# makgyver/gossipy

Hardware: AMD Instinct MI355X
Metric: node-rounds/sec (gossip rounds/sec x nodes, Hegedus-2021 logreg) (higher is better)
Workload: dtype fp32; 1 GPU; model=logreg-57x2 (Hegedus-2021), nodes=1000, nodes_per_gpu=1000, delta=100, protocol=push, mode=merge_update, parallelism=node-sharded gossip over RCCL/xGMI (dp1)

## Files before the change

### gossipy_amd/csrc/scheduler.cpp

```cpp

#include <pybind11/numpy.h>
#include <pybind11/pybind11.h>
#include <pybind11/stl.h>

#include <algorithm>
#include <cmath>
#include <cstdint>
#include <map>
#include <memory>
#include <deque>
#include <functional>
#include <unordered_map>
#include <chrono>
#include <cstdio>
#include <unordered_set>
#include <vector>

#include "round_layout.h"
#include "round_prefetch.h"
#include "round_source.h"

namespace py = pybind11;


// ... 669 lines not shown
        if (ring_mask_) {
            size_t sl = (size_t)t & ring_mask_;
            if (ring_tick_[sl] == t) {
                out.swap(ring_[sl]);
                ring_tick_[sl] = INT64_MIN;
            }
        } else {
            auto it = pending_.find(t);
            if (it != pending_.end()) {
                out = std::move(it->second);
                pending_.erase(it);
            }
        }
        return out;
    }
    int64_t slot_reuse_lag_ = 32;
    std::deque<std::pair<int64_t, int32_t>> reuse_q_;
    int64_t next_slot_ = 0;
    std::vector<int32_t> slot_owner_;

    int32_t alloc_slot(int32_t owner, int64_t t)
    {
        int32_t s;
        if (!reuse_q_.empty() && reuse_q_.front().first + slot_reuse_lag_ <= t) {
            s = reuse_q_.front().second;
            reuse_q_.pop_front();
        } else {
            s = (int32_t)next_slot_++;
            if (next_slot_ > (int64_t)slot_owner_.size())
                slot_owner_.resize(slot_owner_.size() * 2);
// ... 196 lines not shown
    RoundData rd;
    int64_t &sent = rd.sent, &failed = rd.failed, &total_size = rd.total_size;
    auto &snap_nodes = rd.snap_nodes, &snap_slots = rd.snap_slots,
         &snap_tptr = rd.snap_tptr;
    auto &recv_nodes = rd.recv_nodes, &recv_tptr = rd.recv_tptr,
         &recv_nptr = rd.recv_nptr;
    auto &del_slots = rd.del_slots, &del_owners = rd.del_owners,
         &reply_slots = rd.reply_slots, &del_pids = rd.del_pids;
    auto &pull_nodes = rd.pull_nodes, &pull_slots = rd.pull_slots,
         &pull_tptr = rd.pull_tptr;
    auto &rep_nodes = rd.rep_nodes, &rep_tptr = rd.rep_tptr,
         &rep_nptr = rd.rep_nptr;
    auto &rep_slots = rd.rep_slots, &rep_owners = rd.rep_owners,
         &rep_pids = rd.rep_pids;

    std::vector<double> online(n_);
    std::vector<int32_t> firing;
    firing.reserve(64);

    for (int64_t t = t0; t < t1; ++t) {
        std::vector<int32_t> freed;

        firing.clear();
        if (sync_) {
            firing = fire_buckets_[t % delta_];
        } else {
            for (int64_t i = 0; i < n_; ++i)
                if (t % deltas_[i] == 0) firing.push_back((int32_t)i);
        }

        size_t n_f = firing.size();
        if (n_f) {
            Stream gp(stream_key(seed_, PEER, (uint64_t)t, 0));
            std::vector<int32_t> peers(n_f);
            if (indptr_.empty()) {
                for (size_t j = 0; j < n_f; ++j) {
                    int64_t draw = gp.integers(0, n_ - 1);
                    peers[j] = (int32_t)(draw + (draw >= firing[j] ? 1 : 0));
                }
            } else {
                std::vector<double> u(n_f);
                for (size_t j = 0; j < n_f; ++j) u[j] = gp.rnd();
                for (size_t j = 0; j < n_f; ++j) {
                    int64_t s = indptr_[firing[j]];
                    int64_t deg = indptr_[firing[j] + 1] - s;
                    peers[j] = (int32_t)indices_[s + (int64_t)std::floor(
                                                          u[j] * (double)deg)];
                }
            }
            std::vector<double> drop_u(n_f, 1.0);
            if (drop_ > 0.0) {
                Stream gdrop(stream_key(seed_, DROP, (uint64_t)t, 0));
                for (size_t j = 0; j < n_f; ++j) drop_u[j] = gdrop.rnd();
            }
            int64_t msize = (proto_ == PULL) ? 1 : model_size_;
            std::vector<int64_t> delays(n_f);
            {
                Stream gdl(stream_key(seed_, DELAY, (uint64_t)t, 0));
                for (size_t j = 0; j < n_f; ++j) delays[j] = delay_for(gdl, msize);
            }
            std::vector<int32_t> pids(n_f, -1);
            if (n_parts_ > 0) {
                Stream gpt(stream_key(seed_, PART, (uint64_t)t, 0));
                for (size_t j = 0; j < n_f; ++j)
                    pids[j] = (int32_t)gpt.integers(0, n_parts_);
            } else if (sampled_) {
                Stream gsm(stream_key(seed_, SAMPLE, (uint64_t)t, 0));
                for (size_t j = 0; j < n_f; ++j)
                    pids[j] = (int32_t)gsm.integers(0, (int64_t)1 << 31);
            }
            for (size_t j = 0; j < n_f; ++j) {
                int32_t sender = firing[j], receiver = peers[j];
                bool is_pull = proto_ == PULL;
                int32_t slot = -1;
                if (!is_pull) {
                    slot = alloc_slot(sender, t);
                    snap_nodes.push_back(sender);
                    snap_slots.push_back(slot);
                }
                sent += 1;
                total_size += msize;
                if (drop_u[j] >= drop_) {
                    int64_t due = t + delays[j];
                    int32_t rf = (proto_ == PUSH_PULL) ? -2 : -1;
                    pend_push(due, {receiver, slot, rf, is_pull, sender, pids[j]});
                } else {
                    failed += 1;
                    if (slot >= 0) freed.push_back(slot);
                }
            }
        }
        snap_tptr.push_back((int32_t)snap_nodes.size());

        if (online_ < 1.0) {
            Stream go(stream_key(seed_, ONLINE, (uint64_t)t, 0));
            for (int64_t i = 0; i < n_; ++i) online[i] = go.rnd();
        }
        std::vector<Msg> due = pend_take(t);
        std::vector<int32_t> order;
        ev_pool_.clear(); row_head_.clear(); row_tail_.clear();
        const int64_t st_main = 2 * t;
        auto row_append = [&](int64_t stamp, int32_t node, int32_t a,
                              int32_t b, int32_t c, int32_t d) {
            int32_t e = (int32_t)ev_pool_.size();
            ev_pool_.push_back({a, b, c, d, -1});
            if (row_stamp_[node] != stamp) {
                row_stamp_[node] = stamp;
                row_idx_[node] = (int32_t)order.size();
                order.push_back(node);
                row_head_.push_back(e);
                row_tail_.push_back(e);
            } else {
                ev_pool_[row_tail_[row_idx_[node]]].next = e;
                row_tail_[row_idx_[node]] = e;
// ... 27 lines not shown
            freed.push_back(m.slot);
        }
        for (size_t ri = 0; ri < order.size(); ++ri) {
            recv_nodes.push_back(order[ri]);
            for (int32_t e = row_head_[ri]; e >= 0; e = ev_pool_[e].next) {
                del_slots.push_back(ev_pool_[e].v0);
                reply_slots.push_back(ev_pool_[e].v1);
                del_owners.push_back(ev_pool_[e].v2);
                del_pids.push_back(ev_pool_[e].v3);
            }
            recv_nptr.push_back((int32_t)del_slots.size());
        }
        recv_tptr.push_back((int32_t)recv_nodes.size());
        pull_tptr.push_back((int32_t)pull_nodes.size());

        std::vector<Msg> rep_due = pend_take(t);
        std::vector<int32_t> rorder;
        ev_pool_.clear(); row_head_.clear(); row_tail_.clear();
        const int64_t st_rep = 2 * t + 1;
        auto rep_append = [&](int32_t node, int32_t a, int32_t b, int32_t c) {
            int32_t e = (int32_t)ev_pool_.size();
            ev_pool_.push_back({a, b, c, 0, -1});
            if (row_stamp_[node] != st_rep) {
                row_stamp_[node] = st_rep;
                row_idx_[node] = (int32_t)rorder.size();
                rorder.push_back(node);
                row_head_.push_back(e);
                row_tail_.push_back(e);
            } else {
                ev_pool_[row_tail_[row_idx_[node]]].next = e;
                row_tail_[row_idx_[node]] = e;
            }
// ... 9 lines not shown
        }
        for (size_t ri = 0; ri < rorder.size(); ++ri) {
            rep_nodes.push_back(rorder[ri]);
            for (int32_t e = row_head_[ri]; e >= 0; e = ev_pool_[e].next) {
                rep_slots.push_back(ev_pool_[e].v0);
                rep_owners.push_back(ev_pool_[e].v1);
                rep_pids.push_back(ev_pool_[e].v2);
            }
            rep_nptr.push_back((int32_t)rep_slots.size());
        }
        rep_tptr.push_back((int32_t)rep_nodes.size());

        for (int32_t s : freed) reuse_q_.emplace_back(t, s);
    }

    rd.n_slots = next_slot_;
    if (sampling_eval_ > 0) {
        Stream g(stream_key(seed_, EVAL, (uint64_t)(t1 - 1), 0));
        int64_t k = std::max<int64_t>((int64_t)(n_ * sampling_eval_), 1);
        rd.eval_nodes.resize(k);
        for (int64_t i = 0; i < k; ++i) rd.eval_nodes[i] = g.integers(0, n_);
    }
    return rd;
}

void NativeScheduler::pack_generated(RoundData& rd, int64_t n_nodes)
{
    rd.packed = pack_round_compute(
        rd.snap_nodes, rd.snap_slots, rd.snap_tptr, rd.recv_nodes,
        rd.recv_nptr, rd.recv_tptr, rd.del_slots, rd.reply_slots,
// ... 543 lines not shown
```

### gossipy_amd/engine/runner.py

```python

from __future__ import annotations

import os
from typing import List, Optional, Tuple

import numpy as np
import torch
import torch.distributed as dist

from .. import LOG
from ..core import CreateModelMode
from ..simul import SimulationEventSender
from .arena import DataArena, NodeStateArena, SlotPool
from .backend import make_backend
from .metrics import binary_margin_metrics, classification_metrics_shared
from .rng import RandomTape
from .schedule import (
    EngineConfig,
    RoundSchedule,
    Scheduler,
    TickPhase,
    TokenizedScheduler,
    make_scheduler,
)
# ... 1149 lines not shown
            return None
        st, d = self.state, self.data
        key = (
            name, tuple(plan), id(self.scheduler),
            *(t.data_ptr() for t in (st.params, st.ages, d.x, d.y, d.counts,
                                     d.gx, d.gy)),
        )
        if getattr(self, "_rd_key", None) != key:
            self._rd = self.backend.ext.RoundDriver(
                st.params, st.ages, self.pool.slots, self.pool.slot_ages,
                d.x, d.y, d.counts, d.gx, d.gy, name, tuple(plan),
                self.scheduler.round_source(),
                eval_all=not self.cfg.sampling_eval > 0,
                mapped_metrics=env.get("GOSSIPY_RD_NO_MAPPED_EVAL") != "1",
                side_upload=env.get("GOSSIPY_RD_NO_SIDE_UPLOAD") != "1",
            )
            self._rd_key = key
            self._rd_pool = self.pool.slots
        elif self._rd_pool is not self.pool.slots:
            self._rd.set_pool(self.pool.slots, self.pool.slot_ages)
            self._rd_pool = self.pool.slots
        return self._rd

    def _driver_round(self, drv, r: int) -> None:
        res = drv.step(r)
        if res[4] < 0:
            self.pool.ensure(res[3])
            drv.set_pool(self.pool.slots, self.pool.slot_ages)
            self._rd_pool = self.pool.slots
            res = drv.step(r)
# ... 446 lines not shown
```

### gossipy_amd/ops/hip/gossip_kernels.hip

```cpp

#include <torch/extension.h>
#include <pybind11/numpy.h>
#include <ATen/hip/HIPContext.h>
#include <hip/hip_runtime.h>
#include <hip/hip_cooperative_groups.h>

#include <array>
#include <atomic>
#include <chrono>
#include <deque>
#include <stdexcept>
#include <string>
#include <vector>

#include "round_check.h"
#include "round_layout.h"
#include "round_ring.h"
#include "round_source.h"

#define DEV_INLINE __device__ __forceinline__

constexpr int KMAX = 16;
constexpr int WAVE = 64;

// ... 189 lines not shown
            qv[u] = q ? q[s * qs] : 0.f;
        }
        if (q) {
#pragma unroll
            for (int u = 0; u < CH; ++u)
                if (s0 + u < m) g = fmaf(pv[u], qv[u], g);
        } else {
#pragma unroll
            for (int u = 0; u < CH; ++u)
                if (s0 + u < m) g += pv[u];
        }
    }
    return g;
}

template <bool BIG = false>
DEV_INLINE void logreg_update(const LogregArgs& a, int node, int c, float* W,
                              float* xb, float* dz, int& age,
                              int prestaged = 0)
{
    int tid = threadIdx.x;
    if (c == 0) return;
    int bsz = (a.bs == 0) ? c : min(a.bs, c);
    const float* Xn = a.X + (long)node * a.Smax * a.d;
    const float* Yn = a.Y + (long)node * a.Smax;
    int xb_valid = prestaged;
    for (int ep = 0; ep < a.epochs; ++ep) {
        for (int s0 = 0; s0 < c; s0 += bsz) {
            int m = min(bsz, c - s0);
            float yv = (tid < m) ? Yn[s0 + tid] : 0.f;
            if (!xb_valid) copy_row(xb, Xn + (long)s0 * a.d, m * a.d);
            xb_valid = (c <= bsz);
            __syncthreads();
            for (int pr = tid; pr < m * a.k; pr += blockDim.x) {
                int s = pr / a.k, kk = pr - s * a.k;
                dz[pr] = dot_chain(W[a.k * a.d + kk],
                                   W + kk * a.d, xb + s * a.d, a.d);
            }
            __syncthreads();
            auto dz_row = [&](int s, float y) __attribute__((always_inline)) {
                float* zs = dz + s * a.k;
                float amax = -1e30f;
                for (int kk = 0; kk < a.k; ++kk) {
                    float sg = 1.0f / (1.0f + __expf(-zs[kk]));
                    zs[kk] = sg;
                    amax = fmaxf(amax, sg);
                }
                float sum = 0.f;
                for (int kk = 0; kk < a.k; ++kk) sum += __expf(zs[kk] - amax);
                int yi = (int)y;
                float inv = 1.0f / sum;
                for (int kk = 0; kk < a.k; ++kk) {
                    float sg = zs[kk];
                    float pk = __expf(sg - amax);
                    float g = pk * inv - (kk == yi ? 1.0f : 0.0f);
                    zs[kk] = (g / m) * sg * (1.0f - sg);
                }
            };
            if (tid < m) dz_row(tid, yv);
            if constexpr (BIG) {
                for (int s = tid + blockDim.x; s < m; s += blockDim.x)
                    dz_row(s, Yn[s0 + s]);
            }
            __syncthreads();
            for (int e = tid; e < a.k * a.d; e += blockDim.x) {
                int kk = e / a.d, dd = e - kk * a.d;
                float g = col_chain(dz + kk, a.k, xb + dd, a.d, m);
                if (a.wd != 0.f) g += a.wd * W[e];
                W[e] -= a.lr * g;
            }
            for (int e = tid; e < a.k; e += blockDim.x) {
                float g = col_chain(dz + e, a.k, nullptr, 0, m);
                W[a.k * a.d + e] -= a.lr * g;
            }
            __syncthreads();
            age += 1;
        }
    }
}

template <bool LIM, bool BIG = false>
DEV_INLINE void logreg_process_node(const LogregArgs& a, int i)
{
    int node = a.nodes[i];
    int tid = threadIdx.x;
    int c = a.counts[node];
    extern __shared__ float sm[];
    float* W = sm;
    float* W2 = W + a.D;
    float* xb = W2 + a.D;
    int bsmax = (a.bs == 0) ? a.Smax : min(a.bs, a.Smax);
    float* dz = xb + bsmax * a.d;

    int j0 = a.update_only ? 0 : a.ptr[i];
    int j1 = a.update_only ? 0 : a.ptr[i + 1];
    if (!a.update_only && j1 > j0 && a.mode == MODE_MERGE_UPDATE &&
// ... 28 lines not shown
        constexpr int PRE = 8;
        float pre[PRE];
        int pre_age = 0;
        int npre = min(a.D, PRE * (int)blockDim.x);
        auto issue_pre = [&](int j) {
            if (j < j1 && !(a.dmodes && a.dmodes[j])) {
                const float* srow2 = a.slots + (long)a.dslots[j] * a.D;
                for (int u = 0; u < PRE; ++u) {
                    int e = tid + u * (int)blockDim.x;
                    pre[u] = (e < a.D) ? srow2[e] : 0.f;
                }
                pre_age = a.slot_ages[a.dslots[j]];
            }
        };
        issue_pre(j0 + 1);
        logreg_update<BIG>(a, node, c, W, xb, dz, age, 1);
        int rs0 = a.rslots ? a.rslots[j0] : -1;
        if (rs0 >= 0) {
            copy_row(a.slots + (long)rs0 * a.D, W, a.D);
            if (tid == 0) a.slot_ages[rs0] = age;
            __syncthreads();
        }
        for (int j = j0 + 1; j < j1; ++j) {
            int slot2 = a.dslots[j];
            const float* srow2 = a.slots + (long)slot2 * a.D;
            int md = (a.dmodes && a.dmodes[j]) ? MODE_PASS : a.mode;
            if (md == MODE_MERGE_UPDATE) {
                if constexpr (LIM) {
                    LimRule r = lim_rule(age, pre_age, a.lim);
                    if (r.br == LIM_ADOPT) {
                        for (int u = 0; u < PRE; ++u) {
// ... 10 lines not shown
                                   [&](float w, float s) {
                                       return r.m1 * w + r.m2 * s;
                                   });
                    }
                } else {
                    for (int u = 0; u < PRE; ++u) {
                        int e = tid + u * (int)blockDim.x;
                        if (e < a.D) W[e] = 0.5f * (W[e] + pre[u]);
                    }
                    merge_rows(W + npre, srow2 + npre, a.D - npre,
                               [](float w, float s) { return 0.5f * (w + s); });
                }
                age = max(age, pre_age);
                __syncthreads();
                issue_pre(j + 1);
                logreg_update<BIG>(a, node, c, W, xb, dz, age, xb_keep);
            } else {
                copy_row(W, srow2, a.D);
                age = a.slot_ages[slot2];
                __syncthreads();
                issue_pre(j + 1);
            }
            int rs2 = a.rslots ? a.rslots[j] : -1;
            if (rs2 >= 0) {
                copy_row(a.slots + (long)rs2 * a.D, W, a.D);
                if (tid == 0) a.slot_ages[rs2] = age;
                __syncthreads();
            }
        }
        __syncthreads();
        copy_row(a.params + (long)node * a.D, W, a.D);
        if (tid == 0) a.ages[node] = age;
        return;
    }

    copy_row(W, a.params + (long)node * a.D, a.D);
    __syncthreads();
    int age = a.ages[node];

    if (a.update_only) {
        logreg_update<BIG>(a, node, c, W, xb, dz, age);
    } else {
        for (int j = a.ptr[i]; j < a.ptr[i + 1]; ++j) {
            int slot = a.dslots[j];
            const float* srow = a.slots + (long)slot * a.D;
            int sage = a.slot_ages[slot];
            int md = (a.dmodes && a.dmodes[j]) ? MODE_PASS : a.mode;
            if (md == MODE_MERGE_UPDATE) {
                if constexpr (LIM) {
                    lim_merge_row(lim_rule(age, sage, a.lim), W, srow, a.D);
                } else {
                    merge_rows(W, srow, a.D, [](float w, float s) {
                        return 0.5f * (w + s);
                    });
                }
                age = max(age, sage);
                __syncthreads();
                logreg_update<BIG>(a, node, c, W, xb, dz, age);
            } else if (md == MODE_UPDATE) {
                copy_row(W, srow, a.D);
                age = sage;
                __syncthreads();
                logreg_update<BIG>(a, node, c, W, xb, dz, age);
            } else if (md == MODE_UPDATE_MERGE) {
                logreg_update<BIG>(a, node, c, W, xb, dz, age);
                copy_row(W2, srow, a.D);
                __syncthreads();
                int age2 = sage;
                logreg_update<BIG>(a, node, c, W2, xb, dz, age2);
                if constexpr (LIM) {
                    lim_merge_row(lim_rule(age, age2, a.lim), W, W2, a.D);
                } else {
                    for (int e = tid; e < a.D; e += blockDim.x)
                        W[e] = 0.5f * (W[e] + W2[e]);
                }
                age = max(age, age2);
                __syncthreads();
            } else {
                copy_row(W, srow, a.D);
                age = sage;
                __syncthreads();
            }
            int rs = a.rslots ? a.rslots[j] : -1;
            if (rs >= 0) {
// ... 18 lines not shown
tick_logreg_lim_kernel(LogregArgs a)
{
    logreg_process_node<true>(a, blockIdx.x);
}

__global__ void __launch_bounds__(128)
tick_logreg_big_kernel(LogregArgs a)
{
    logreg_process_node<false, true>(a, blockIdx.x);
}

__global__ void __launch_bounds__(128)
tick_logreg_lim_big_kernel(LogregArgs a)
{
    logreg_process_node<true, true>(a, blockIdx.x);
}


__global__ void wmerge_kernel(
    float* __restrict__ params,
    int* __restrict__ ages,
    const float* __restrict__ slots,
    const int* __restrict__ slot_ages,
    const int* __restrict__ nodes,
    const int* __restrict__ ptr,
    const int* __restrict__ wslots,
    const float* __restrict__ wweights,
    const float* __restrict__ selfw,
    int D)
{
// ... 1649 lines not shown
    int D = params.size(1);
    hipLaunchKernelGGL(wmerge_kernel, dim3(n), dim3(128), 0, current_stream(),
        params.data_ptr<float>(), ages.data_ptr<int>(),
        slots.data_ptr<float>(), slot_ages.data_ptr<int>(),
        nodes.data_ptr<int>(), ptr.data_ptr<int>(),
        wslots.numel() ? wslots.data_ptr<int>() : nullptr,
        wweights.numel() ? wweights.data_ptr<float>() : nullptr,
        selfw.data_ptr<float>(), D);
}


template <typename Args>
struct Plan {
    Args a{};
    void (*kernel)(Args) = nullptr;
    size_t smem = 0;
    int threads = 0;
    SnapGeom snap{};
};

template <typename Args>
struct channel {
    using type = const int* Args::*;
};

struct StateTensors {
    torch::Tensor params, ages, slots, slot_ages, X, Y, counts;
};

template <typename A>
static void fill_state_x(A& a, const StateTensors& st)
{
    const torch::Tensor &params = st.params, &slots = st.slots, &X = st.X;
    CHECK_DEV(params); CHECK_DEV(slots); CHECK_DEV(X);
// ... 16 lines not shown
static void fill_sgd(A& a, double lr, double wd, int64_t epochs, int64_t bs,
                     int64_t mode)
{
    a.lr = lr; a.wd = wd; a.epochs = epochs; a.bs = bs; a.mode = mode;
}

static int batch_rows(int64_t bs, int Smax)
{
    return (bs == 0) ? Smax : std::min<int>(bs, Smax);
}

constexpr int LOGREG_THREADS = 128;
static bool big_batch(int64_t bs, int Smax)
{
    return batch_rows(bs, Smax) > LOGREG_THREADS;
}

static int check_merge_limit(int64_t merge_limit)
{
    TORCH_CHECK(merge_limit >= -1 && merge_limit <= (1 << 30),
                "merge_limit must be -1 (off) or in [0, 2^30], got ",
                merge_limit);
    return (int)std::max<int64_t>(merge_limit, 0);
}

template <typename A> static A& events(A& a) { return a; }
static MlpArgs& events(MlpCompArgs& c) { return c.m; }

static Plan<LogregArgs> logreg_plan(
    const StateTensors& st, int64_t d, int64_t k, double lr, double wd,
    int64_t epochs, int64_t bs, int64_t mode, int64_t merge_limit = -1)
{
    Plan<LogregArgs> L;
    LogregArgs& a = L.a;
    fill_state(a, st);
    TORCH_CHECK(k <= KMAX, "n_classes > ", KMAX, " unsupported");
    a.d = d; a.k = k; a.D = st.params.size(1);
    fill_sgd(a, lr, wd, epochs, bs, mode);
    a.lim = check_merge_limit(merge_limit);
    int bsmax = batch_rows(bs, a.Smax);
    L.smem = sizeof(float) * (2 * a.D + (size_t)bsmax * a.d + (size_t)bsmax * a.k);
    TORCH_CHECK(L.smem <= 160 * 1024, "logreg LDS budget exceeded: ", L.smem);
    if (big_batch(bs, a.Smax))
        L.kernel = (merge_limit >= 0) ? tick_logreg_lim_big_kernel
                                      : tick_logreg_big_kernel;
    else
        L.kernel = (merge_limit >= 0) ? tick_logreg_lim_kernel
                                      : tick_logreg_kernel;
    L.threads = LOGREG_THREADS;
    L.snap = {a.D, a.D, 0, 1};
    return L;
}

static Plan<LinearArgs> linear_plan(
    const StateTensors& st, int64_t d, double lrlam, int64_t is_pegasos,
    int64_t mode)
{
    Plan<LinearArgs> L;
    LinearArgs& a = L.a;
    fill_state(a, st);
    TORCH_CHECK(d <= LIN_MAX_REGS * WAVE, "d > ", LIN_MAX_REGS * WAVE, " unsupported");
    a.d = d;
    a.lrlam = lrlam; a.is_pegasos = is_pegasos; a.mode = mode;
    L.kernel = tick_linear_kernel;
// ... 204 lines not shown

template <typename Args>
static void launch_tick(Plan<Args>& L, const TickEvents& ev, bool update_only,
                        typename channel<Args>::type chan = nullptr,
                        const torch::Tensor& chan_vals = {})
{
    const torch::Tensor &nodes = ev.nodes, &recv_ptr = ev.recv_ptr;
    int n = nodes.size(0);
    if (n == 0) return;
    CHECK_DEV(nodes); CHECK_DEV(recv_ptr);
    auto& e = events(L.a);
    e.nodes = nodes.data_ptr<int>(); e.ptr = recv_ptr.data_ptr<int>();
    e.dslots = iptr(ev.del_slots); e.rslots = iptr(ev.reply_slots);
    e.update_only = update_only;
    if (chan) L.a.*chan = iptr(chan_vals);
    launch_kernel(L.kernel, n, L.threads, L.smem, current_stream(), L.a);
}

void tick_logreg(torch::Tensor params, torch::Tensor ages, torch::Tensor slots,
                 torch::Tensor slot_ages, torch::Tensor nodes, torch::Tensor recv_ptr,
                 torch::Tensor del_slots, torch::Tensor reply_slots,
                 torch::Tensor X, torch::Tensor Y, torch::Tensor counts,
                 int64_t d, int64_t k, double lr, double wd, int64_t epochs,
                 int64_t bs, int64_t mode, int64_t merge_limit,
                 bool update_only, torch::Tensor dmodes)
{
    auto L = logreg_plan({params, ages, slots, slot_ages, X, Y, counts},
                         d, k, lr, wd, epochs, bs, mode, merge_limit);
    launch_tick(L, {nodes, recv_ptr, del_slots, reply_slots}, update_only,
                &LogregArgs::dmodes, dmodes);
}
// ... 136 lines not shown

template <typename Args>
static void stream_round(Plan<Args>& L, const RoundArrays& r,
                         typename channel<Args>::type chan = nullptr)
{
    hipStream_t s = current_stream();
    auto& e = events(L.a);
    auto snap = [&](const int* nodes, const int* slot_ids, int n) {
        launch_snap(e.params, e.ages, e.slots, e.slot_ages, nodes, slot_ids,
                    n, L.snap, s);
    };
    auto deliver = [&](const int* nodes, const int* nptr, int n,
                       const int* dslots, const int* rslots, const int* pids) {
        e.nodes = nodes; e.ptr = nptr; e.dslots = dslots; e.rslots = rslots;
        if (chan) L.a.*chan = pids;
        launch_kernel(L.kernel, n, L.threads, L.smem, s, L.a);
    };
    const int* const* a = r.dev;
    for (int t = 0; t < r.delta; ++t) {
        int s0 = r.tptr[RT_SNAP][t], s1 = r.tptr[RT_SNAP][t + 1];
        if (s1 > s0)
            snap(a[RA_SNAP_NODES] + s0, a[RA_SNAP_SLOTS] + s0, s1 - s0);
        int r0 = r.tptr[RT_RECV][t], r1 = r.tptr[RT_RECV][t + 1];
        if (r1 > r0)
            deliver(a[RA_RECV_NODES] + r0, a[RA_RECV_NPTR] + r0, r1 - r0,
                    a[RA_DEL_SLOTS], a[RA_REPLY_SLOTS], a[RA_DEL_PIDS]);
        int p0 = r.tptr[RT_PULL][t], p1 = r.tptr[RT_PULL][t + 1];
        if (p1 > p0)
            snap(a[RA_PULL_NODES] + p0, a[RA_PULL_SLOTS] + p0, p1 - p0);
        int q0 = r.tptr[RT_REP][t], q1 = r.tptr[RT_REP][t + 1];
        if (q1 > q0)
// ... 373 lines not shown
    (void)hipEventDestroy(e);
}

static py::tuple round_driver_live()
{
    return py::make_tuple(rd_live[RD_HOST].load(), rd_live[RD_DEV].load(),
                          rd_live[RD_EVENT].load(), rd_live[RD_STREAM].load());
}

class RoundDriver {
public:
    RoundDriver(torch::Tensor params, torch::Tensor ages, torch::Tensor slots,
                torch::Tensor slot_ages, torch::Tensor X, torch::Tensor Y,
                torch::Tensor counts, torch::Tensor gx, torch::Tensor gy,
                const std::string& family, py::tuple plan, py::capsule source,
                bool eval_all, bool mapped_metrics, bool side_upload)
        : st_{params, ages, slots, slot_ages, X, Y, counts}, gx_(gx), gy_(gy),
          source_cap_(source), eval_all_(eval_all), mapped_(mapped_metrics),
          side_upload_(side_upload)
    {
        TORCH_CHECK(std::string(source.name() ? source.name() : "") ==
                        "gossipy_amd.RoundSource",
                    "source must be NativeScheduler.round_source()");
        src_ = *static_cast<const RoundSource*>(source.get_pointer());
        CHECK_DEV(gx); CHECK_DEV(gy);
        if (family == "logreg") {
            TORCH_CHECK(plan.size() == 8,
                        "logreg plan: (d, k, lr, wd, epochs, bs, mode,"
                        " merge_limit)");
            lg_ = logreg_plan(
                st_, plan[0].cast<int64_t>(), plan[1].cast<int64_t>(),
                plan[2].cast<double>(), plan[3].cast<double>(),
                plan[4].cast<int64_t>(), plan[5].cast<int64_t>(),
                plan[6].cast<int64_t>(), plan[7].cast<int64_t>());
// ... 35 lines not shown
        ev_.eval_counts = nullptr;
        ev_smem_ = eval_tile_smem(ev_);
        n_local_ = params.size(0);
        pool_cap_ = slots.size(0);
        try {
            for (auto& s : ring_)
                rd_event_create(&s.ev);
            for (auto& m : stage_)
                rd_event_create(&m.ev);
            if (side_upload_) {
                RD_CHECK(hipStreamCreateWithFlags(&up_stream_,
                                                  hipStreamNonBlocking));
                ++rd_live[RD_STREAM];
                rd_event_create(&up_ev_);
            }
        } catch (...) {
            release();
            throw;
        }
    }

    RoundDriver(const RoundDriver&) = delete;
    RoundDriver& operator=(const RoundDriver&) = delete;

    ~RoundDriver() { release(); }

    void set_pool(torch::Tensor slots, torch::Tensor slot_ages)
    {
        check_pool(slots, slot_ages);
        st_.slots = slots; st_.slot_ages = slot_ages;
// ... 79 lines not shown

    py::list drain() { return poll_eval(true); }

private:
    struct Slot {
        int32_t* h = nullptr;
        int32_t* d = nullptr;
        size_t cap = 0;
        hipEvent_t ev = nullptr;
    };
    struct Stage {
        float* h = nullptr;
        float* h_dev = nullptr;
        size_t cap_rows = 0;
        hipEvent_t ev = nullptr;
        int64_t round = 0;
        int64_t rows = 0;
    };
    struct Done {
        int64_t round, rows;
        std::vector<float> vals;
    };

    const SnapGeom& snap_geom() const { return linear_ ? ln_.snap : lg_.snap; }

    void check_pool(const torch::Tensor& slots,
                    const torch::Tensor& slot_ages) const
    {
        const SnapGeom& g = snap_geom();
        TORCH_CHECK(slots.is_cuda() && slots.is_contiguous() &&
// ... 36 lines not shown
        s.d = nullptr;
        rd_host_alloc((void**)&s.h, cap * sizeof(int32_t), hipHostMallocDefault);
        rd_dev_alloc((void**)&s.d, cap * sizeof(int32_t));
        s.cap = cap;
    }

    void grow_stage(Stage& m, size_t rows)
    {
        size_t cap = grown_capacity(m.cap_rows, rows);
        if (cap == m.cap_rows) return;
        if (m.h) RD_CHECK(rd_host_free(m.h));
        m.h = nullptr; m.cap_rows = 0;
        rd_host_alloc((void**)&m.h, cap * 5 * sizeof(float), hipHostMallocMapped);
        RD_CHECK(hipHostGetDevicePointer((void**)&m.h_dev, m.h, 0));
        m.cap_rows = cap;
    }

    int64_t run_held()
    {
        hipStream_t s = current_stream();
        const RoundView& v = view_;
        int64_t n_ids_max = (int64_t)v.n_eval;
        bool will_eval = n_ids_max > 0 || eval_all_;
        if (will_eval && pending_.size() >= 2) collect_oldest();

        int si = slots_.acquire(
            [&](int i) {
                hipError_t q = hipEventQuery(ring_[i].ev);
                if (q != hipErrorNotReady) RD_CHECK(q);
                return q == hipSuccess;
// ... 35 lines not shown
                                      : (eval_all_ ? n_local_ : 0);
            if (rows) {
                int mi = stage_next_;
                Stage& m = stage_[mi];
                grow_stage(m, (size_t)rows);
                if (!mapped_ && (size_t)rows > d_out_rows_) {
                    size_t cap = grown_capacity(d_out_rows_, (size_t)rows);
                    if (d_out_) RD_CHECK(rd_dev_free(d_out_));
                    d_out_ = nullptr; d_out_rows_ = 0;
                    rd_dev_alloc((void**)&d_out_, cap * 5 * sizeof(float));
                    d_out_rows_ = cap;
                }
                EvalArgs a = ev_;
                a.nodes = lay.n_eval ? sl.d + lay.eval_off : nullptr;
                a.out = mapped_ ? m.h_dev : d_out_;
                launch_kernel(eval_metrics_kernel, (int)rows, 256, ev_smem_,
                              s, a);
                if (!mapped_)
                    RD_CHECK(hipMemcpyAsync(m.h, d_out_,
                                            (size_t)rows * 5 * sizeof(float),
                                            hipMemcpyDeviceToHost, s));
                RD_CHECK(hipEventRecord(m.ev, s));
                m.round = held_r_; m.rows = rows;
                pending_.push_back(mi);
                stage_next_ ^= 1;
            }
            RD_CHECK(hipEventRecord(sl.ev, s));
            recorded = true;
            return rows;
        } catch (...) {
            if (!recorded) {
                (void)hipStreamSynchronize(s);
                if (side_upload_) (void)hipStreamSynchronize(up_stream_);
                slots_.abandon(si);
            }
            throw;
        }
    }

    void release() noexcept
    {
        for (auto& s : ring_) {
            if (s.ev) { (void)hipEventSynchronize(s.ev); rd_event_destroy(s.ev); }
            if (s.h) (void)rd_host_free(s.h);
            if (s.d) (void)rd_dev_free(s.d);
            s = Slot{};
        }
        for (auto& m : stage_) {
            if (m.ev) { (void)hipEventSynchronize(m.ev); rd_event_destroy(m.ev); }
            if (m.h) (void)rd_host_free(m.h);
            m = Stage{};
        }
        if (d_out_) (void)rd_dev_free(d_out_);
        d_out_ = nullptr;
        if (up_ev_) rd_event_destroy(up_ev_);
        if (up_stream_) {
            (void)hipStreamSynchronize(up_stream_);
            (void)hipStreamDestroy(up_stream_);
            --rd_live[RD_STREAM];
        }
        up_ev_ = nullptr; up_stream_ = nullptr;
    }

    StateTensors st_;
    torch::Tensor gx_, gy_;
    py::capsule source_cap_;
    RoundSource src_{};
    bool eval_all_, mapped_, side_upload_;
    bool linear_ = false;
    Plan<LogregArgs> lg_;
    Plan<LinearArgs> ln_;
    EvalArgs ev_{};
    size_t ev_smem_ = 0;
    int64_t n_local_ = 0, pool_cap_ = 0;

    RoundView view_{};
    bool held_ = false, failed_ = false;
    int64_t held_r_ = -1, last_groups_ = 0, rounds_ = 0;
    double take_s_ = 0, enqueue_s_ = 0;

    Slot ring_[RD_RING];
    SlotRing<RD_RING> slots_;
    Stage stage_[2];
    int stage_next_ = 0;
    std::deque<int> pending_;
    std::vector<Done> done_;
    float* d_out_ = nullptr;
    size_t d_out_rows_ = 0;
    hipStream_t up_stream_ = nullptr;
    hipEvent_t up_ev_ = nullptr;
};

PYBIND11_MODULE(TORCH_EXTENSION_NAME, m)
{
    py::class_<RoundDriver>(m, "RoundDriver")
        .def(py::init<torch::Tensor, torch::Tensor, torch::Tensor,
                      torch::Tensor, torch::Tensor, torch::Tensor,
                      torch::Tensor, torch::Tensor, torch::Tensor,
                      const std::string&, py::tuple, py::capsule, bool, bool,
                      bool>(),
             py::arg("params"), py::arg("ages"), py::arg("slots"),
             py::arg("slot_ages"), py::arg("X"), py::arg("Y"),
             py::arg("counts"), py::arg("gx"), py::arg("gy"),
             py::arg("family"), py::arg("plan"), py::arg("source"),
             py::arg("eval_all") = false, py::arg("mapped_metrics") = true,
             py::arg("side_upload") = true)
        .def("step", &RoundDriver::step)
        .def("set_pool", &RoundDriver::set_pool)
        .def("poll_eval", &RoundDriver::poll_eval)
        .def("drain", &RoundDriver::drain)
        .def("stats", &RoundDriver::stats)
        .def_property_readonly("last_groups", &RoundDriver::last_groups);
    m.def("round_driver_live", &round_driver_live,
          "(pinned host buffers, device buffers, events, streams) held by "
          "the RoundDrivers of this process");
    m.def("snapshot", &snapshot, "batched model snapshot (arena row copy)");
    py::tuple arrays((size_t)ROUND_N_ARRAYS), tptrs((size_t)ROUND_N_TPTRS);
    for (int i = 0; i < ROUND_N_ARRAYS; ++i) arrays[i] = ROUND_ARRAY_NAMES[i];
    for (int i = 0; i < ROUND_N_TPTRS; ++i) tptrs[i] = ROUND_TPTR_NAMES[i];
    m.attr("ROUND_ARRAY_NAMES") = arrays;
    m.attr("ROUND_TPTR_NAMES") = tptrs;
// ... 52 lines not shown
```

Before: 9.216 million node-rounds/s.

## Reuse scheduler scratch buffers, add pipelined thin logreg kernels, optional eval overlap

The host scheduler now keeps its per-tick vectors in a persistent scratch struct and pre-reserves the round output arrays from the previous round's sizes, removing repeated heap allocation in generate_round. New 'thin' logreg kernel variants use a software-pipelined dot product and a register-based softmax for k=2. They are picked when the node count per launch is below a CU-derived threshold, meant for small per-tick launches. A third change, off by default, gathers eval rows into a private buffer and runs evaluation on a separate stream to overlap it with the next round's ticks, at the cost of extra memory and another stream.

Measured after the change: 9.835 million node-rounds/s, median of 6. 6.7% higher.

```diff
diff --git a/gossipy_amd/csrc/scheduler.cpp b/gossipy_amd/csrc/scheduler.cpp
--- a/gossipy_amd/csrc/scheduler.cpp
+++ b/gossipy_amd/csrc/scheduler.cpp
@@ -707,6 +707,30 @@
         }
         return out;
     }
+    void pend_take_into(int64_t t, std::vector<Msg>& out)
+    {
+        out.clear();
+        if (ring_mask_) {
+            size_t sl = (size_t)t & ring_mask_;
+            if (ring_tick_[sl] == t) {
+                out.swap(ring_[sl]);
+                ring_tick_[sl] = INT64_MIN;
+            }
+        } else {
+            auto it = pending_.find(t);
+            if (it != pending_.end()) {
+                out = std::move(it->second);
+                pending_.erase(it);
+            }
+        }
+    }
+    struct TickScratch {
+        std::vector<int32_t> firing, freed, peers, pids, order, rorder;
+        std::vector<double> online, u, drop_u;
+        std::vector<int64_t> delays;
+        std::vector<Msg> due, rep_due;
+        size_t snap = 0, recv = 0, del = 0, pull = 0, rep = 0, rep_del = 0;
+    } sc_;
     int64_t slot_reuse_lag_ = 32;
     std::deque<std::pair<int64_t, int32_t>> reuse_q_;
     int64_t next_slot_ = 0;
@@ -933,32 +957,49 @@
     auto &rep_slots = rd.rep_slots, &rep_owners = rd.rep_owners,
          &rep_pids = rd.rep_pids;
 
-    std::vector<double> online(n_);
-    std::vector<int32_t> firing;
-    firing.reserve(64);
+    const size_t n_ticks = (size_t)delta_ + 1;
+    snap_nodes.reserve(sc_.snap); snap_slots.reserve(sc_.snap);
+    snap_tptr.reserve(n_ticks);
+    recv_nodes.reserve(sc_.recv); recv_nptr.reserve(sc_.recv + 1);
+    recv_tptr.reserve(n_ticks);
+    del_slots.reserve(sc_.del); del_owners.reserve(sc_.del);
+    reply_slots.reserve(sc_.del); del_pids.reserve(sc_.del);
+    pull_nodes.reserve(sc_.pull); pull_slots.reserve(sc_.pull);
+    pull_tptr.reserve(n_ticks);
+    rep_nodes.reserve(sc_.rep); rep_nptr.reserve(sc_.rep + 1);
+    rep_tptr.reserve(n_ticks);
+    rep_slots.reserve(sc_.rep_del); rep_owners.reserve(sc_.rep_del);
+    rep_pids.reserve(sc_.rep_del);
+
+    auto &online = sc_.online, &u = sc_.u, &drop_u = sc_.drop_u;
+    auto &freed = sc_.freed, &peers = sc_.peers, &pids = sc_.pids,
+         &order = sc_.order, &rorder = sc_.rorder;
+    auto& delays = sc_.delays;
+    auto &due = sc_.due, &rep_due = sc_.rep_due;
+    if (online_ < 1.0) online.resize((size_t)n_);
 
     for (int64_t t = t0; t < t1; ++t) {
-        std::vector<int32_t> freed;
-
-        firing.clear();
-        if (sync_) {
-            firing = fire_buckets_[t % delta_];
-        } else {
+        freed.clear();
+
+        if (!sync_) {
+            sc_.firing.clear();
             for (int64_t i = 0; i < n_; ++i)
-                if (t % deltas_[i] == 0) firing.push_back((int32_t)i);
-        }
+                if (t % deltas_[i] == 0) sc_.firing.push_back((int32_t)i);
+        }
+        const std::vector<int32_t>& firing =
+            sync_ ? fire_buckets_[t % delta_] : sc_.firing;
 
         size_t n_f = firing.size();
         if (n_f) {
             Stream gp(stream_key(seed_, PEER, (uint64_t)t, 0));
-            std::vector<int32_t> peers(n_f);
+            peers.resize(n_f);
             if (indptr_.empty()) {
                 for (size_t j = 0; j < n_f; ++j) {
                     int64_t draw = gp.integers(0, n_ - 1);
                     peers[j] = (int32_t)(draw + (draw >= firing[j] ? 1 : 0));
                 }
             } else {
-                std::vector<double> u(n_f);
+                u.resize(n_f);
                 for (size_t j = 0; j < n_f; ++j) u[j] = gp.rnd();
                 for (size_t j = 0; j < n_f; ++j) {
                     int64_t s = indptr_[firing[j]];
@@ -967,18 +1008,18 @@
                                                           u[j] * (double)deg)];
                 }
             }
-            std::vector<double> drop_u(n_f, 1.0);
+            drop_u.assign(n_f, 1.0);
             if (drop_ > 0.0) {
                 Stream gdrop(stream_key(seed_, DROP, (uint64_t)t, 0));
                 for (size_t j = 0; j < n_f; ++j) drop_u[j] = gdrop.rnd();
             }
             int64_t msize = (proto_ == PULL) ? 1 : model_size_;
-            std::vector<int64_t> delays(n_f);
+            delays.resize(n_f);
             {
                 Stream gdl(stream_key(seed_, DELAY, (uint64_t)t, 0));
                 for (size_t j = 0; j < n_f; ++j) delays[j] = delay_for(gdl, msize);
             }
-            std::vector<int32_t> pids(n_f, -1);
+            pids.assign(n_f, -1);
             if (n_parts_ > 0) {
                 Stream gpt(stream_key(seed_, PART, (uint64_t)t, 0));
                 for (size_t j = 0; j < n_f; ++j)
@@ -1000,9 +1041,9 @@
                 sent += 1;
                 total_size += msize;
                 if (drop_u[j] >= drop_) {
-                    int64_t due = t + delays[j];
+                    int64_t due_t = t + delays[j];
                     int32_t rf = (proto_ == PUSH_PULL) ? -2 : -1;
-                    pend_push(due, {receiver, slot, rf, is_pull, sender, pids[j]});
+                    pend_push(due_t, {receiver, slot, rf, is_pull, sender, pids[j]});
                 } else {
                     failed += 1;
                     if (slot >= 0) freed.push_back(slot);
@@ -1015,8 +1056,8 @@
             Stream go(stream_key(seed_, ONLINE, (uint64_t)t, 0));
             for (int64_t i = 0; i < n_; ++i) online[i] = go.rnd();
         }
-        std::vector<Msg> due = pend_take(t);
-        std::vector<int32_t> order;
+        pend_take_into(t, due);
+        order.clear();
         ev_pool_.clear(); row_head_.clear(); row_tail_.clear();
         const int64_t st_main = 2 * t;
         auto row_append = [&](int64_t stamp, int32_t node, int32_t a,
@@ -1074,8 +1115,8 @@
         recv_tptr.push_back((int32_t)recv_nodes.size());
         pull_tptr.push_back((int32_t)pull_nodes.size());
 
-        std::vector<Msg> rep_due = pend_take(t);
-        std::vector<int32_t> rorder;
+        pend_take_into(t, rep_due);
+        rorder.clear();
         ev_pool_.clear(); row_head_.clear(); row_tail_.clear();
         const int64_t st_rep = 2 * t + 1;
         auto rep_append = [&](int32_t node, int32_t a, int32_t b, int32_t c) {
@@ -1115,6 +1156,9 @@
         for (int32_t s : freed) reuse_q_.emplace_back(t, s);
     }
 
+    sc_.snap = snap_nodes.size(); sc_.recv = recv_nodes.size();
+    sc_.del = del_slots.size(); sc_.pull = pull_nodes.size();
+    sc_.rep = rep_nodes.size(); sc_.rep_del = rep_slots.size();
     rd.n_slots = next_slot_;
     if (sampling_eval_ > 0) {
         Stream g(stream_key(seed_, EVAL, (uint64_t)(t1 - 1), 0));
diff --git a/gossipy_amd/engine/runner.py b/gossipy_amd/engine/runner.py
--- a/gossipy_amd/engine/runner.py
+++ b/gossipy_amd/engine/runner.py
@@ -1187,6 +1187,7 @@
                 eval_all=not self.cfg.sampling_eval > 0,
                 mapped_metrics=env.get("GOSSIPY_RD_NO_MAPPED_EVAL") != "1",
                 side_upload=env.get("GOSSIPY_RD_NO_SIDE_UPLOAD") != "1",
+                eval_overlap=env.get("GOSSIPY_RD_EVAL_OVERLAP") == "1",
             )
             self._rd_key = key
             self._rd_pool = self.pool.slots
diff --git a/gossipy_amd/ops/hip/gossip_kernels.hip b/gossipy_amd/ops/hip/gossip_kernels.hip
--- a/gossipy_amd/ops/hip/gossip_kernels.hip
+++ b/gossipy_amd/ops/hip/gossip_kernels.hip
@@ -227,7 +227,106 @@
     return g;
 }
 
-template <bool BIG = false>
+DEV_INLINE float dot_chain_pipe(float acc, const float* w, const float* x, int d)
+{
+    float wa[CH], xa[CH], wb[CH], xb[CH];
+    auto load = [&](float* wv, float* xv, int e) __attribute__((always_inline)) {
+#pragma unroll
+        for (int u = 0; u < CH; ++u) { wv[u] = w[e + u]; xv[u] = x[e + u]; }
+    };
+    auto fma = [&](const float* wv, const float* xv) __attribute__((always_inline)) {
+#pragma unroll
+        for (int u = 0; u < CH; ++u) acc = fmaf(wv[u], xv[u], acc);
+    };
+    int e0 = 0;
+    if (CH <= d) load(wa, xa, 0);
+    for (; e0 + 3 * CH <= d; e0 += 2 * CH) {
+        load(wb, xb, e0 + CH);
+        __builtin_amdgcn_sched_barrier(0);
+        fma(wa, xa);
+        __builtin_amdgcn_sched_barrier(0);
+        load(wa, xa, e0 + 2 * CH);
+        __builtin_amdgcn_sched_barrier(0);
+        fma(wb, xb);
+        __builtin_amdgcn_sched_barrier(0);
+    }
+    if (e0 + 2 * CH <= d) {
+        load(wb, xb, e0 + CH);
+        fma(wa, xa);
+        fma(wb, xb);
+        e0 += 2 * CH;
+    } else if (e0 + CH <= d) {
+        fma(wa, xa);
+        e0 += CH;
+    }
+    int r = d - e0;
+#pragma unroll
+    for (int u = 0; u < CH - 1; ++u) {
+        if (u >= r) break;
+        wb[u] = w[e0 + u]; xb[u] = x[e0 + u];
+    }
+#pragma unroll
+    for (int u = 0; u < CH - 1; ++u) {
+        if (u >= r) break;
+        acc = fmaf(wb[u], xb[u], acc);
+        asm volatile("" : "+v"(acc));
+    }
+    return acc;
+}
+
+template <bool Q = true>
+DEV_INLINE float col_chain_exact(const float* p, int ps, const float* q, int qs,
+                           int m)
+{
+    m = __builtin_amdgcn_readfirstlane(m);
+    float g = 0.f;
+    for (int s0 = 0; s0 < m; s0 += CH) {
+        float pv[CH], qv[CH];
+        int r = min(CH, m - s0);
+#pragma unroll
+        for (int u = 0; u < CH; ++u) {
+            if (u >= r) break;
+            pv[u] = p[(s0 + u) * ps];
+            if constexpr (Q) qv[u] = q[(s0 + u) * qs];
+        }
+#pragma unroll
+        for (int u = 0; u < CH; ++u) {
+            if (u >= r) break;
+            if constexpr (Q) g = fmaf(pv[u], qv[u], g); else g += pv[u];
+            asm volatile("" : "+v"(g));
+        }
+    }
+    return g;
+}
+
+template <int K>
+DEV_INLINE void dz_row_regs(float* zs, float y, int m)
+{
+    float sg[K], pk[K];
+#pragma unroll
+    for (int kk = 0; kk < K; ++kk) sg[kk] = zs[kk];
+    float amax = -1e30f;
+#pragma unroll
+    for (int kk = 0; kk < K; ++kk) {
+        sg[kk] = 1.0f / (1.0f + __expf(-sg[kk]));
+        amax = fmaxf(amax, sg[kk]);
+    }
+    float sum = 0.f;
+#pragma unroll
+    for (int kk = 0; kk < K; ++kk) {
+        pk[kk] = __expf(sg[kk] - amax);
+        sum += pk[kk];
+    }
+    int yi = (int)y;
+    float inv = 1.0f / sum;
+#pragma unroll
+    for (int kk = 0; kk < K; ++kk) {
+        float g = pk[kk] * inv - (kk == yi ? 1.0f : 0.0f);
+        zs[kk] = (g / m) * sg[kk] * (1.0f - sg[kk]);
+    }
+}
+
+template <bool BIG = false, bool PIPE = false>
 DEV_INLINE void logreg_update(const LogregArgs& a, int node, int c, float* W,
                               float* xb, float* dz, int& age,
                               int prestaged = 0)
@@ -247,12 +346,21 @@
             __syncthreads();
             for (int pr = tid; pr < m * a.k; pr += blockDim.x) {
                 int s = pr / a.k, kk = pr - s * a.k;
-                dz[pr] = dot_chain(W[a.k * a.d + kk],
-                                   W + kk * a.d, xb + s * a.d, a.d);
+                const float* wk = W + kk * a.d;
+                const float* xs = xb + s * a.d;
+                float bias = W[a.k * a.d + kk];
+                if constexpr (PIPE) dz[pr] = dot_chain_pipe(bias, wk, xs, a.d);
+                else dz[pr] = dot_chain(bias, wk, xs, a.d);
             }
             __syncthreads();
             auto dz_row = [&](int s, float y) __attribute__((always_inline)) {
                 float* zs = dz + s * a.k;
+                if constexpr (PIPE) {
+                    if (a.k == 2) {
+                        dz_row_regs<2>(zs, y, m);
+                        return;
+                    }
+                }
                 float amax = -1e30f;
                 for (int kk = 0; kk < a.k; ++kk) {
                     float sg = 1.0f / (1.0f + __expf(-zs[kk]));
@@ -278,12 +386,16 @@
             __syncthreads();
             for (int e = tid; e < a.k * a.d; e += blockDim.x) {
                 int kk = e / a.d, dd = e - kk * a.d;
-                float g = col_chain(dz + kk, a.k, xb + dd, a.d, m);
+                float g = PIPE
+                    ? col_chain_exact<true>(dz + kk, a.k, xb + dd, a.d, m)
+                    : col_chain(dz + kk, a.k, xb + dd, a.d, m);
                 if (a.wd != 0.f) g += a.wd * W[e];
                 W[e] -= a.lr * g;
             }
             for (int e = tid; e < a.k; e += blockDim.x) {
-                float g = col_chain(dz + e, a.k, nullptr, 0, m);
+                float g = PIPE
+                    ? col_chain_exact<false>(dz + e, a.k, nullptr, 0, m)
+                    : col_chain(dz + e, a.k, nullptr, 0, m);
                 W[a.k * a.d + e] -= a.lr * g;
             }
             __syncthreads();
@@ -292,7 +404,7 @@
     }
 }
 
-template <bool LIM, bool BIG = false>
+template <bool LIM, bool BIG = false, bool PIPE = false>
 DEV_INLINE void logreg_process_node(const LogregArgs& a, int i)
 {
     int node = a.nodes[i];
@@ -351,7 +463,7 @@
             }
         };
         issue_pre(j0 + 1);
-        logreg_update<BIG>(a, node, c, W, xb, dz, age, 1);
+        logreg_update<BIG, PIPE>(a, node, c, W, xb, dz, age, 1);
         int rs0 = a.rslots ? a.rslots[j0] : -1;
         if (rs0 >= 0) {
             copy_row(a.slots + (long)rs0 * a.D, W, a.D);
@@ -392,7 +504,7 @@
                 age = max(age, pre_age);
                 __syncthreads();
                 issue_pre(j + 1);
-                logreg_update<BIG>(a, node, c, W, xb, dz, age, xb_keep);
+                logreg_update<BIG, PIPE>(a, node, c, W, xb, dz, age, xb_keep);
             } else {
                 copy_row(W, srow2, a.D);
                 age = a.slot_ages[slot2];
@@ -417,7 +529,7 @@
     int age = a.ages[node];
 
     if (a.update_only) {
-        logreg_update<BIG>(a, node, c, W, xb, dz, age);
+        logreg_update<BIG, PIPE>(a, node, c, W, xb, dz, age);
     } else {
         for (int j = a.ptr[i]; j < a.ptr[i + 1]; ++j) {
             int slot = a.dslots[j];
@@ -434,18 +546,18 @@
                 }
                 age = max(age, sage);
                 __syncthreads();
-                logreg_update<BIG>(a, node, c, W, xb, dz, age);
+                logreg_update<BIG, PIPE>(a, node, c, W, xb, dz, age);
             } else if (md == MODE_UPDATE) {
                 copy_row(W, srow, a.D);
                 age = sage;
                 __syncthreads();
-                logreg_update<BIG>(a, node, c, W, xb, dz, age);
+                logreg_update<BIG, PIPE>(a, node, c, W, xb, dz, age);
             } else if (md == MODE_UPDATE_MERGE) {
-                logreg_update<BIG>(a, node, c, W, xb, dz, age);
+                logreg_update<BIG, PIPE>(a, node, c, W, xb, dz, age);
                 copy_row(W2, srow, a.D);
                 __syncthreads();
                 int age2 = sage;
-                logreg_update<BIG>(a, node, c, W2, xb, dz, age2);
+                logreg_update<BIG, PIPE>(a, node, c, W2, xb, dz, age2);
                 if constexpr (LIM) {
                     lim_merge_row(lim_rule(age, age2, a.lim), W, W2, a.D);
                 } else {
@@ -494,6 +606,30 @@
 tick_logreg_lim_big_kernel(LogregArgs a)
 {
     logreg_process_node<true, true>(a, blockIdx.x);
+}
+
+__global__ void __launch_bounds__(128)
+tick_logreg_thin_kernel(LogregArgs a)
+{
+    logreg_process_node<false, false, true>(a, blockIdx.x);
+}
+
+__global__ void __launch_bounds__(128)
+tick_logreg_lim_thin_kernel(LogregArgs a)
+{
+    logreg_process_node<true, false, true>(a, blockIdx.x);
+}
+
+__global__ void __launch_bounds__(128)
+tick_logreg_big_thin_kernel(LogregArgs a)
+{
+    logreg_process_node<false, true, true>(a, blockIdx.x);
+}
+
+__global__ void __launch_bounds__(128)
+tick_logreg_lim_big_thin_kernel(LogregArgs a)
+{
+    logreg_process_node<true, true, true>(a, blockIdx.x);
 }
 
 
@@ -2173,10 +2309,18 @@
 struct Plan {
     Args a{};
     void (*kernel)(Args) = nullptr;
+    void (*kernel_thin)(Args) = nullptr;
+    int thin_rows = 0;
     size_t smem = 0;
     int threads = 0;
     SnapGeom snap{};
 };
+
+template <typename Args>
+static auto plan_kernel(const Plan<Args>& L, int n)
+{
+    return (L.kernel_thin && n <= L.thin_rows) ? L.kernel_thin : L.kernel;
+}
 
 template <typename Args>
 struct channel {
@@ -2223,6 +2367,18 @@
 static bool big_batch(int64_t bs, int Smax)
 {
     return batch_rows(bs, Smax) > LOGREG_THREADS;
+}
+
+static int thin_launch_rows(int threads)
+{
+    int dev = 0, cus = 0;
+    hipError_t err = hipGetDevice(&dev);
+    if (err == hipSuccess)
+        err = hipDeviceGetAttribute(
+            &cus, hipDeviceAttributeMultiprocessorCount, dev);
+    TORCH_CHECK(err == hipSuccess, "device query failed: ",
+                hipGetErrorString(err));
+    return cus * 4 / std::max(1, threads / WAVE);
 }
 
 static int check_merge_limit(int64_t merge_limit)
@@ -2250,13 +2406,18 @@
     int bsmax = batch_rows(bs, a.Smax);
     L.smem = sizeof(float) * (2 * a.D + (size_t)bsmax * a.d + (size_t)bsmax * a.k);
     TORCH_CHECK(L.smem <= 160 * 1024, "logreg LDS budget exceeded: ", L.smem);
-    if (big_batch(bs, a.Smax))
-        L.kernel = (merge_limit >= 0) ? tick_logreg_lim_big_kernel
-                                      : tick_logreg_big_kernel;
-    else
-        L.kernel = (merge_limit >= 0) ? tick_logreg_lim_kernel
-                                      : tick_logreg_kernel;
+    bool lim = merge_limit >= 0;
+    if (big_batch(bs, a.Smax)) {
+        L.kernel = lim ? tick_logreg_lim_big_kernel : tick_logreg_big_kernel;
+        L.kernel_thin = lim ? tick_logreg_lim_big_thin_kernel
+                            : tick_logreg_big_thin_kernel;
+    } else {
+        L.kernel = lim ? tick_logreg_lim_kernel : tick_logreg_kernel;
+        L.kernel_thin = lim ? tick_logreg_lim_thin_kernel
+                            : tick_logreg_thin_kernel;
+    }
     L.threads = LOGREG_THREADS;
+    L.thin_rows = thin_launch_rows(LOGREG_THREADS);
     L.snap = {a.D, a.D, 0, 1};
     return L;
 }
@@ -2491,7 +2652,8 @@
     e.dslots = iptr(ev.del_slots); e.rslots = iptr(ev.reply_slots);
     e.update_only = update_only;
     if (chan) L.a.*chan = iptr(chan_vals);
-    launch_kernel(L.kernel, n, L.threads, L.smem, current_stream(), L.a);
+    launch_kernel(plan_kernel(L, n), n, L.threads, L.smem, current_stream(),
+                  L.a);
 }
 
 void tick_logreg(torch::Tensor params, torch::Tensor ages, torch::Tensor slots,
@@ -2658,7 +2820,7 @@
                        const int* dslots, const int* rslots, const int* pids) {
         e.nodes = nodes; e.ptr = nptr; e.dslots = dslots; e.rslots = rslots;
         if (chan) L.a.*chan = pids;
-        launch_kernel(L.kernel, n, L.threads, L.smem, s, L.a);
+        launch_kernel(plan_kernel(L, n), n, L.threads, L.smem, s, L.a);
     };
     const int* const* a = r.dev;
     for (int t = 0; t < r.delta; ++t) {
@@ -3062,10 +3224,11 @@
                 torch::Tensor slot_ages, torch::Tensor X, torch::Tensor Y,
                 torch::Tensor counts, torch::Tensor gx, torch::Tensor gy,
                 const std::string& family, py::tuple plan, py::capsule source,
-                bool eval_all, bool mapped_metrics, bool side_upload)
+                bool eval_all, bool mapped_metrics, bool side_upload,
+                bool eval_overlap)
         : st_{params, ages, slots, slot_ages, X, Y, counts}, gx_(gx), gy_(gy),
           source_cap_(source), eval_all_(eval_all), mapped_(mapped_metrics),
-          side_upload_(side_upload)
+          side_upload_(side_upload), eval_overlap_(eval_overlap)
     {
         TORCH_CHECK(std::string(source.name() ? source.name() : "") ==
                         "gossipy_amd.RoundSource",
@@ -3131,6 +3294,13 @@
                 ++rd_live[RD_STREAM];
                 rd_event_create(&up_ev_);
             }
+            if (eval_overlap_) {
+                RD_CHECK(hipStreamCreateWithFlags(&ev_stream_,
+                                                  hipStreamNonBlocking));
+                ++rd_live[RD_STREAM];
+                for (auto& m : stage_)
+                    rd_event_create(&m.gev);
+            }
         } catch (...) {
             release();
             throw;
@@ -3240,6 +3410,9 @@
         float* h_dev = nullptr;
         size_t cap_rows = 0;
         hipEvent_t ev = nullptr;
+        float* rows_d = nullptr;
+        size_t rows_cap = 0;
+        hipEvent_t gev = nullptr;
         int64_t round = 0;
         int64_t rows = 0;
     };
@@ -3306,6 +3479,28 @@
         rd_host_alloc((void**)&m.h, cap * 5 * sizeof(float), hipHostMallocMapped);
         RD_CHECK(hipHostGetDevicePointer((void**)&m.h_dev, m.h, 0));
         m.cap_rows = cap;
+    }
+
+    void grow_gather(Stage& m, size_t rows, hipStream_t s)
+    {
+        size_t cap = grown_capacity(m.rows_cap, rows);
+        if (cap != m.rows_cap) {
+            if (m.rows_d) RD_CHECK(rd_dev_free(m.rows_d));
+            m.rows_d = nullptr; m.rows_cap = 0;
+            rd_dev_alloc((void**)&m.rows_d, cap * ev_.D * sizeof(float));
+            m.rows_cap = cap;
+        }
+        if (cap > ident_cap_) {
+            RD_CHECK(hipStreamSynchronize(s));
+            if (ident_d_) RD_CHECK(rd_dev_free(ident_d_));
+            ident_d_ = nullptr; ident_cap_ = 0;
+            rd_dev_alloc((void**)&ident_d_, cap * sizeof(int));
+            std::vector<int> iota(cap);
+            for (size_t i = 0; i < cap; ++i) iota[i] = (int)i;
+            RD_CHECK(hipMemcpy(ident_d_, iota.data(), cap * sizeof(int),
+                               hipMemcpyHostToDevice));
+            ident_cap_ = cap;
+        }
     }
 
     int64_t run_held()
@@ -3371,21 +3566,37 @@
                 EvalArgs a = ev_;
                 a.nodes = lay.n_eval ? sl.d + lay.eval_off : nullptr;
                 a.out = mapped_ ? m.h_dev : d_out_;
+                hipStream_t es = s;
+                if (eval_overlap_ && lay.n_eval) {
+                    grow_gather(m, (size_t)rows, s);
+                    launch_snap(ev_.params, nullptr, m.rows_d, nullptr,
+                                a.nodes, ident_d_, (int)rows,
+                                SnapGeom{ev_.D, ev_.D, 0, 0}, s);
+                    RD_CHECK(hipGetLastError());
+                    RD_CHECK(hipEventRecord(m.gev, s));
+                    RD_CHECK(hipEventRecord(sl.ev, s));
+                    recorded = true;
+                    es = ev_stream_;
+                    RD_CHECK(hipStreamWaitEvent(es, m.gev, 0));
+                    a.params = m.rows_d;
+                    a.nodes = nullptr;
+                }
                 launch_kernel(eval_metrics_kernel, (int)rows, 256, ev_smem_,
-                              s, a);
+                              es, a);
                 if (!mapped_)
                     RD_CHECK(hipMemcpyAsync(m.h, d_out_,
                                             (size_t)rows * 5 * sizeof(float),
-                                            hipMemcpyDeviceToHost, s));
-                RD_CHECK(hipEventRecord(m.ev, s));
+                                            hipMemcpyDeviceToHost, es));
+                RD_CHECK(hipEventRecord(m.ev, es));
                 m.round = held_r_; m.rows = rows;
                 pending_.push_back(mi);
                 stage_next_ ^= 1;
             }
-            RD_CHECK(hipEventRecord(sl.ev, s));
+            if (!recorded) RD_CHECK(hipEventRecord(sl.ev, s));
             recorded = true;
             return rows;
         } catch (...) {
+            if (ev_stream_) (void)hipStreamSynchronize(ev_stream_);
             if (!recorded) {
                 (void)hipStreamSynchronize(s);
                 if (side_upload_) (void)hipStreamSynchronize(up_stream_);
@@ -3403,11 +3614,24 @@
             if (s.d) (void)rd_dev_free(s.d);
             s = Slot{};
         }
+        if (ev_stream_) (void)hipStreamSynchronize(ev_stream_);
         for (auto& m : stage_) {
             if (m.ev) { (void)hipEventSynchronize(m.ev); rd_event_destroy(m.ev); }
+            if (m.gev) {
+                (void)hipEventSynchronize(m.gev);
+                rd_event_destroy(m.gev);
+            }
             if (m.h) (void)rd_host_free(m.h);
+            if (m.rows_d) (void)rd_dev_free(m.rows_d);
             m = Stage{};
         }
+        if (ident_d_) (void)rd_dev_free(ident_d_);
+        ident_d_ = nullptr; ident_cap_ = 0;
+        if (ev_stream_) {
+            (void)hipStreamDestroy(ev_stream_);
+            --rd_live[RD_STREAM];
+        }
+        ev_stream_ = nullptr;
         if (d_out_) (void)rd_dev_free(d_out_);
         d_out_ = nullptr;
         if (up_ev_) rd_event_destroy(up_ev_);
@@ -3423,7 +3647,7 @@
     torch::Tensor gx_, gy_;
     py::capsule source_cap_;
     RoundSource src_{};
-    bool eval_all_, mapped_, side_upload_;
+    bool eval_all_, mapped_, side_upload_, eval_overlap_;
     bool linear_ = false;
     Plan<LogregArgs> lg_;
     Plan<LinearArgs> ln_;
@@ -3446,6 +3670,9 @@
     size_t d_out_rows_ = 0;
     hipStream_t up_stream_ = nullptr;
     hipEvent_t up_ev_ = nullptr;
+    hipStream_t ev_stream_ = nullptr;
+    int* ident_d_ = nullptr;
+    size_t ident_cap_ = 0;
 };
 
 PYBIND11_MODULE(TORCH_EXTENSION_NAME, m)
@@ -3455,13 +3682,13 @@
                       torch::Tensor, torch::Tensor, torch::Tensor,
                       torch::Tensor, torch::Tensor, torch::Tensor,
                       const std::string&, py::tuple, py::capsule, bool, bool,
-                      bool>(),
+                      bool, bool>(),
              py::arg("params"), py::arg("ages"), py::arg("slots"),
              py::arg("slot_ages"), py::arg("X"), py::arg("Y"),
              py::arg("counts"), py::arg("gx"), py::arg("gy"),
              py::arg("family"), py::arg("plan"), py::arg("source"),
              py::arg("eval_all") = false, py::arg("mapped_metrics") = true,
-             py::arg("side_upload") = true)
+             py::arg("side_upload") = true, py::arg("eval_overlap") = false)
         .def("step", &RoundDriver::step)
         .def("set_pool", &RoundDriver::set_pool)
         .def("poll_eval", &RoundDriver::poll_eval)
```
